# al-mcintyre/mCaller

Measured on AMD Instinct MI355X. Metric: m6A calls/sec (GATC motif, E. coli-like synthetic eventalign), higher is better.
Workload: dtype f64 (K1 window means, everything written); K2 hidden layer f32 + f64 output + f64 re-evaluation near print boundaries (MCALLER_MLP_FP64=1 = f64 throughout: ms_per_step_fp64_mlp); 1 GPU; synthetic 1e+08 eventalign rows per GPU and step, -m GATC, NN classifier (r95 two-base MLP), skip_thresh 0; two resident tables taken in turn, every step a FULL pass (the table declared new: positions + event indices streamed, every row validated); step=full pass, passes_in_flight=4, events_per_gpu=100000000, flush_records_per_gpu=204194, copy_out_bytes_per_pass=8767737

## Files before the change

### include/mcaller_hip.h

```cpp
#ifndef MCALLER_HIP_H
#define MCALLER_HIP_H

#define MC_E_NO_FREE_SLOT (-16)

#include <stdint.h>

#ifdef __cplusplus
extern "C" {
#endif

#define MC_MAX_K 8

#define MC_F_KMER_EQ    0x01
#define MC_F_MODEL_N    0x02
#define MC_F_SEG_START  0x04
#define MC_F_NAME_START 0x08

typedef struct mc_table_view {
    int64_t n_rows;
    const int32_t *pos;
    const int32_t *event_model_e4;
    const int32_t *event_idx;
    const uint8_t *flags;
    int32_t n_seg;
// ... 90 lines not shown
int mc_fastq_read_quality(const char *path, int32_t n_threads, mc_fastq **out);
int64_t mc_fastq_view(const mc_fastq *f, const char **key_pool, const int64_t **key_off, const double **mean);
void mc_fastq_free(mc_fastq *f);

typedef struct mc_ctx mc_ctx;
int mc_ctx_create(int device, mc_ctx **out);
int mc_bind_to_device_numa_node(int device);
void mc_ctx_destroy(mc_ctx *ctx);
int mc_ctx_set_reference(mc_ctx *ctx, const mc_ref_view *host_ref);
int mc_ctx_set_reference_motif(mc_ctx *ctx, const mc_ref_view *host_ref, const char *motif_fwd, const char *repl_fwd, int32_t m_fwd,
                               const char *motif_rev, const char *repl_rev, int32_t m_rev);
int mc_ctx_set_reference_iupac(mc_ctx *ctx, const mc_ref_view *host_ref, const mc_iupac_spec *spec);
int mc_ctx_fetch_reference(mc_ctx *ctx, uint8_t *seq, int64_t n_seq_bytes, uint32_t *mbits_fwd, uint32_t *mbits_rev,
                           int32_t *rank_fwd, int32_t *rank_rev, int64_t n_words, int64_t *site_base, int64_t *n_sites);
int mc_ctx_upload_table(mc_ctx *ctx, const mc_table_view *host_table);
int mc_ctx_set_read_quality(mc_ctx *ctx, const double *qual, int32_t n_reads);

#define MC_TABLE_SLOTS 12
int mc_ctx_reserve_tables(mc_ctx *ctx, int64_t max_rows, int32_t max_segs, int32_t max_reads);
int mc_ctx_upload_table_async(mc_ctx *ctx, const mc_table_view *host_table, const double *read_qual, int32_t *slot);
int mc_ctx_wait_upload(mc_ctx *ctx, int32_t slot);
int mc_ctx_current_slot(mc_ctx *ctx);
int mc_ctx_select_table(mc_ctx *ctx, int32_t slot, int32_t as_new);
int mc_ctx_upload_times_ms(mc_ctx *ctx, int32_t slot, float *h2d_ms, float *validate_ms);
int mc_ctx_parse_times_ms(mc_ctx *ctx, int32_t slot, float *text_h2d_ms, float *parse_ms);
int mc_ctx_set_mlp(mc_ctx *ctx, int32_t n_models, int32_t n_in, int32_t n_hidden,
                   const double *W1, const double *b1, const double *W2, const double *b2,
                   const uint8_t *submodel_of_char);

int mc_ctx_set_forest(mc_ctx *ctx, int32_t n_models, int32_t n_in, const int32_t *model_tree_off,
                      const int32_t *tree_node_off, const int32_t *left, const int32_t *right, const int32_t *feature,
                      const double *threshold, const double *value, const uint8_t *submodel_of_char);

#define MC_CLF_LOGISTIC 1
#define MC_CLF_GNB 2
int mc_ctx_set_simple_classifier(mc_ctx *ctx, int32_t kind, int32_t n_models, int32_t n_in, const double *params, int32_t stride,
                                 const uint8_t *submodel_of_char);

int mc_ctx_set_svm(mc_ctx *ctx, int32_t n_models, int32_t n_in, const int32_t *model_sv_off, const double *sv,
                   const double *dual_coef, const double *params, const uint8_t *submodel_of_char);

typedef struct mc_params {
    int32_t k;
    int32_t skip_thresh;
    double  qual_thresh;
    int32_t tail_contig;
    int32_t score;
    int32_t entry_read;
    int32_t entry_first_idx;
} mc_params;

int mc_last_pass_info(mc_ctx *ctx, int32_t *fused_room, int32_t *rerun);
int mc_ctx_last_scan_mode(mc_ctx *ctx);
int mc_ctx_row_text(mc_ctx *ctx, int32_t on, const char *label_meth, const char *label_unmeth);
int mc_last_row_text(mc_ctx *ctx, const char **text, int64_t *n_bytes, int64_t *n_rows, int32_t *block);
int mc_row_text_release(mc_ctx *ctx, int32_t block);
#define MC_ROWTEXT_PROBE_STRIDE 48
int mc_ctx_rowtext_probe(mc_ctx *ctx, const double *v, int64_t n, const int32_t *fixed, int64_t n_fixed, const double *prob, int64_t n_prob,
                         int32_t shift, char *text, int32_t *len, uint8_t *ok);
int mc_extract_features(mc_ctx *ctx, const mc_params *prm, int64_t *n_records);
int mc_fetch_records(mc_ctx *ctx, const mc_calls_view *host_out);
int mc_fetch_records_view(mc_ctx *ctx, mc_calls_view *out);
int mc_extract_features_async(mc_ctx *ctx, const mc_params *prm);
int mc_wait_records(mc_ctx *ctx, int64_t *n_records, mc_calls_view *out);
int mc_wait_records_begin(mc_ctx *ctx);
int mc_last_times_ms(mc_ctx *ctx, float *out5);
int mc_ctx_set_pass_timing(mc_ctx *ctx, int every_n);
int mc_last_pass_timed(mc_ctx *ctx);
int mc_ctx_sync(mc_ctx *ctx);

int mc_mlp_forward(mc_ctx *ctx, const double *X, const uint8_t *submodel, int64_t n, double *p);
int mc_forest_forward(mc_ctx *ctx, const double *X, const uint8_t *submodel, int64_t n, double *p);
int mc_simple_forward(mc_ctx *ctx, const double *X, const uint8_t *submodel, int64_t n, double *p);
int mc_svm_forward(mc_ctx *ctx, const double *X, const uint8_t *submodel, int64_t n, double *p);

#define MC_UNIQUE_ID_BYTES 128
int64_t mc_site_count(mc_ctx *ctx);
int mc_site_counts(mc_ctx *ctx, int64_t row_offset, int32_t tail_contig, int64_t *n_pending, int64_t *n_cross_contig);
int mc_site_counts_reset(mc_ctx *ctx);
int mc_site_counts_accumulate(mc_ctx *ctx, int64_t row_offset, int32_t tail_contig, int64_t *n_pending, int64_t *n_cross_contig);
int mc_site_counts_add(mc_ctx *ctx, const int64_t *site, const uint8_t *is_meth, const int64_t *first_row, int64_t n);
int mc_comm_available(void);
int mc_comm_unique_id(uint8_t *out128);
int mc_comm_init(mc_ctx *ctx, int32_t world, int32_t rank, const uint8_t *unique_id128);
int mc_comm_destroy(mc_ctx *ctx);
int mc_site_allreduce(mc_ctx *ctx, int32_t *n_meth, int32_t *n_total, int64_t *first_row, float *ms);
int mc_site_counts_fetch(mc_ctx *ctx, int32_t *n_meth, int32_t *n_total, int64_t *first_row);

typedef struct mc_fit_params {
    int32_t n_in, n_hidden;
    int32_t batch_size;
    int32_t max_iter;
    int32_t n_iter_no_change;
    int32_t shuffle;
    double alpha, lr_init, beta1, beta2, epsilon, tol;
    uint64_t seed;
} mc_fit_params;
int mc_mlp_fit(mc_ctx *ctx, const mc_fit_params *prm, const double *X, const uint8_t *y, int64_t n_samples, int32_t n_jobs,
               const int64_t *train_off, const int32_t *train_idx, const int64_t *val_off, const int32_t *val_idx,
               const uint64_t *seeds, const double *init,
               double *W1, double *b1, double *W2, double *b2,
               double *loss_curve , int32_t *n_iter , int64_t *val_correct);

typedef struct mc_forest_params {
    int32_t n_in;
    int32_t n_trees;
// ... 538 lines not shown
```

### mcaller_amd/csrc/mc_dev.h

```cpp
#ifndef MC_DEV_H
#define MC_DEV_H
#include <hip/hip_runtime.h>
#include <hip/hip_ext.h>
#include <sched.h>

#include <algorithm>
#include <cctype>
#include <chrono>
#include <cmath>
#include <cstdio>
#include <cstdlib>
#include <cstring>
#include <type_traits>
#include <vector>

#include "../../include/mcaller_hip.h"

void mc_set_error(const char *fmt, ...);

#define HIP_TRY(expr)                                                                       \
    do {                                                                                    \
        hipError_t _e = (expr);                                                             \
        if (_e != hipSuccess) {                                                             \
            mc_set_error("%s failed: %s (%s:%d)", #expr, hipGetErrorString(_e), __FILE__, __LINE__); \
// ... 289 lines not shown
    const NbDesc *desc;
    Payload *payload;
    long long payload_cap;
    long long *tile_chunk;
    int chunk_shift;
    int shard_shift;
    int shard_mask;
    int32_t *tile_cnt;
    int32_t *tile_half;
    const int32_t *tile_local;
    const int64_t *group_sum;
    int64_t *tile_first;
    DevRecords O;
    Counters *cnt;
    int k, skip_thresh, tail_contig;
    int64_t *rare_list;
    unsigned long long pass_no;
    int32_t *piece_cnt;
    int32_t *piece_kw;
    unsigned long long *chunk_cnt;
};

__device__ __forceinline__ int64_t find_close(const DevTable &T, const NbDesc *__restrict__ desc, int tail_contig,
                                              int nb_abs, int64_t my_end, int64_t r, int &close_pos, bool &close_ns) {
    int64_t rr = r + 1;
    int bb = nb_abs;
    close_ns = false;
    close_pos = 0;
    while (rr < T.n_rows) {
        if (rr < my_end) {
            if (!(T.flags[rr] & MC_F_MODEL_N)) { close_pos = T.pos[rr]; return rr; }
            ++rr;
            continue;
        }
        close_ns = true;
        while (bb + 1 < T.n_nb && T.nb_row_begin[bb + 1] <= rr) ++bb;
        if (desc[bb].filtered) { rr = T.nb_row_begin[bb + 1]; continue; }
        if (!(T.flags[rr] & MC_F_MODEL_N)) { close_pos = T.pos[rr]; return rr; }
        ++rr;
    }
    close_ns = true;
    return tail_contig >= 0 ? T.n_rows : -1;
}

constexpr int PT = 16;
constexpr int NCHUNK = TILE / 64 + 1;
#ifndef MC_CHUNK
#define MC_CHUNK 1024
#endif
constexpr int CHUNK = MC_CHUNK;
constexpr int NCH = TILE / CHUNK;
constexpr int NQ = CHUNK / 512;
static_assert(CHUNK % 512 == 0 && TILE % CHUNK == 0, "whole stripes, whole chunks");

constexpr int GROUP = 1024;

__device__ __forceinline__ int64_t tile_slot(const int32_t *__restrict__ tile_local, const int64_t *__restrict__ group_sum,
                                             int64_t tile, int lane) {
    const int g = (int)(tile / GROUP);
    long long part = 0;
    for (int i = lane; i < g; i += 64) part += group_sum[i];
    for (int o = 32; o > 0; o >>= 1) part += __shfl_xor(part, o);
    return part + tile_local[tile];
}

constexpr int EG = 8;
constexpr int K2_MAXM = 8;

struct PackLayout { size_t pos, seg, info, feats; };
__host__ __device__ inline PackLayout pack_layout(int64_t n, int close32) {
    PackLayout L;
    L.pos = (size_t)n * (close32 ? 4 : 8);
    L.seg = L.pos + (size_t)n * 4;
    L.info = L.seg + (size_t)n * 4;
    L.feats = (L.info + (size_t)n * 4 + 7) & ~(size_t)7;
    return L;
}

struct PackTail { size_t lo32, prob, wmask, hi32, end; };
__host__ __device__ inline PackTail pack_tail(size_t feats_off, size_t m, int k, size_t n_wide) {
    PackTail T;
    T.lo32 = feats_off;
    T.prob = (T.lo32 + m * (size_t)k * 4 + 7) & ~(size_t)7;
    T.wmask = T.prob + m * 8;
    T.hi32 = (T.wmask + m + 3) & ~(size_t)3;
    T.end = T.hi32 + n_wide * 4;
    return T;
}

struct LitArgs {
    DevTable T;
    DevRef R;
    const NbDesc *desc;
    const int64_t *nb_f0;
    const double *qual;
    double qual_thresh;
    int k, skip_thresh, tail_contig, entry_read, entry_first_idx;
    int32_t *run_cnt;
    int32_t *run_rows;
    const int32_t *cnt_local;
    const int64_t *cnt_group;
    const int32_t *rows_local;
    const int64_t *rows_group;
    double *scratch;
    DevRecords L;
    int write;
// ... 90 lines not shown
```

### mcaller_amd/csrc/mc_scan.hip

```cpp
#include "mc_dev.h"

namespace {

__global__ __launch_bounds__(256) void k_unit_columns(DevTable T) {
    const int64_t g4 = blockIdx.x * (int64_t)256 + threadIdx.x;
    const bool have = g4 * 4 < T.n_rows;
    int4 p = make_int4(0, 0, 0, 0);
    if (have) {
        p = *reinterpret_cast<const int4 *>(T.pos + g4 * 4);
        reinterpret_cast<int32_t *>(T.unit_pp)[g4] = (g4 & 1) ? p.w : p.x;
    }
    int before = __shfl_up(p.w, 1);
    if ((threadIdx.x & 63) == 0 && have && g4 > 0) before = T.pos[g4 * 4 - 1];
    const int ps[5] = {before, p.x, p.y, p.z, p.w};
    uint32_t dec = 0, zero = 0;
#pragma unroll
    for (int e = 0; e < 4; ++e) {
        const int64_t r = g4 * 4 + e;
        const bool in = r < T.n_rows;
        dec |= (in && r > 0 && ps[e + 1] < ps[e] ? 1u : 0u) << e;
        zero |= (in && ps[e + 1] == 0 ? 1u : 0u) << e;
    }
    const uint32_t mine = dec | (zero << 8);
    const uint32_t other = __shfl_down(mine, 1);
// ... 207 lines not shown
__device__ __forceinline__ NbDesc desc_uniform(const NbDesc *desc, int b) {
    const NbDesc *p = uniform_ptr(desc) + __builtin_amdgcn_readfirstlane(b);
    union { u32x16 w; NbDesc d; } u;
    asm volatile("s_load_dwordx16 %0, %1, 0x0\n\ts_waitcnt lgkmcnt(0)" : "=s"(u.w) : "s"(p));
    return u.d;
}
__device__ __forceinline__ int64_t desc_row_end_uniform(const NbDesc *desc, int b) {
    const int64_t *p = &(uniform_ptr(desc) + __builtin_amdgcn_readfirstlane(b))->row_end;
    int64_t v;
    asm volatile("s_load_dwordx2 %0, %1, 0x0\n\ts_waitcnt lgkmcnt(0)" : "=s"(v) : "s"(p));
    return v;
}

template <int MODE> constexpr bool summary_cols() { return MODE == SCAN_SUMMARY || MODE == SCAN_VALIDATE_SUMMARY; }
template <int MODE> constexpr bool validating() { return MODE == SCAN_VALIDATE || MODE == SCAN_VALIDATE_SUMMARY; }
template <int MODE> constexpr bool nbits_streamed() { return !summary_cols<MODE>(); }
static_assert(MC_F_MODEL_N == 2, "flag_bytes(): where the bit goes in the flag byte");
__device__ __forceinline__ uint32_t flag_bytes(uint32_t b4) { return (((b4 & 0xFu) * 0x00204081u) & 0x01010101u) << 1; }

template <int MODE>
struct ChunkCols {
    int4 pa[NQ], pb[NQ];
    uint32_t xr[NQ];
    uint32_t pr[NQ];
    uint32_t nb[NQ];
    __device__ __forceinline__ void load(const DevTable &T, int64_t c0, int crows, int lane) {
#pragma unroll
        for (int j = 0; j < NQ; ++j) {
            const int i0 = (j * 64 + lane) * 8;
            pa[j] = pb[j] = make_int4(0, 0, 0, 0);
            xr[j] = pr[j] = 0u;
            nb[j] = 0xFFu;
            if (i0 < crows) {
                if (summary_cols<MODE>()) {
                    const int2 pp = T.unit_pp[(c0 + i0) >> 3];
                    pa[j].x = pp.x;
                    pb[j].w = pp.y;
                    if (MODE == SCAN_VALIDATE_SUMMARY) {
                        xr[j] = T.xrel[(c0 + i0) >> 3];
                        pr[j] = T.prel[(c0 + i0) >> 3];
                    }
                } else {
                    pa[j] = *reinterpret_cast<const int4 *>(T.pos + c0 + i0);
                    pb[j] = *reinterpret_cast<const int4 *>(T.pos + c0 + i0 + 4);
                    nb[j] = T.nbits[(c0 + i0) >> 3];
                    if (MODE == SCAN_VALIDATE) {
                        xr[j] = T.xrel[(c0 + i0) >> 3];
                    }
                }
            }
        }
    }
};

struct DenseStash { const int4 *pa, *pb, *fw; const int *dec; };
__device__ __forceinline__ void dense_block_rows(const K1Args &A, TileSlots &S, long long &ahead, DenseStash L, int nb_abs, int64_t c0,
                                                 int64_t c1, int2 tail_p, uint32_t tail_f) {
    const DevTable &T = A.T;
    const int lane = threadIdx.x, k = A.k;
    const unsigned long long below = (1ull << lane) - 1ull;
    const uint32_t kmask = (1u << k) - 1u;
    ScanGlobals G;
    G.pos = T.pos; G.flags = T.flags; G.nb_row_begin = T.nb_row_begin; G.desc = A.desc; G.n_rows = T.n_rows;
    G.n_nb = T.n_nb; G.tail_contig = A.tail_contig; G.k = k; G.skip_thresh = A.skip_thresh;
    const NbDesc d = desc_uniform(A.desc, nb_abs);
    if (d.mode != MODE_REGULAR) return;
    const uint32_t *gbits = (d.rev ? A.R.mr : A.R.mf) + d.mask_off;
    if (d.extra_row() >= c0 && d.extra_row() < c1) {
        const CloseRes xc = far_close_body(G, nb_abs, d.row_end, d.extra_row());
        Payload P;
        P.r = d.extra_row(); P.close_row = xc.row; P.m = d.extra_mpos; P.close_pos = xc.pos;
        P.flags = PF_EXTRA | (xc.ns ? PF_CLOSE_NS : 0u);
        P.nb = nb_abs;
        S.put(lane == 0 && xc.row >= 0, P, &ahead);
    }
    const int64_t lb_abs = max(d.row_begin, d.first());
    const int lo = (int)(max(lb_abs, c0) - c0), hi = (int)(min(d.row_end, c1) - c0);
    const int hi_close = (int)(min(d.row_end, c1 + 2) - c0);
    const uint32_t base_flags = (d.stray_q != NO_STRAY ? PF_STRAY : 0u) | (d.rev ? PF_REV : 0u);
#pragma unroll 1
    for (int j = 0; j < NQ; ++j) {
        if (j * 512 + 512 <= lo || j * 512 >= hi) continue;
        const int i0 = (j * 64 + lane) * 8;
        const int4 qa = L.pa[j * 64 + lane], qb = L.pb[j * 64 + lane], qw = L.fw[j * 64 + lane];
        const int un = j * 64 + lane + 1;
        const bool last = un >= NQ * 64;
        const int4 na = L.pa[last ? 0 : un], nw = L.fw[last ? 0 : un];
        const int nx = last ? tail_p.x : na.x, ny = last ? tail_p.y : na.y;
        const uint32_t nf = last ? tail_f : (uint32_t)nw.x;
        const int ps[10] = {qa.x, qa.y, qa.z, qa.w, qb.x, qb.y, qb.z, qb.w, nx, ny};
        const uint32_t nbits = ((uint32_t)qw.x & 0xFFu) | ((nf & 3u) << 8);
        const uint32_t below_hi = (1u << min(max(hi - i0, 0), 10)) - 1u, from_lo = ~((1u << min(max(lo - i0, 0), 10)) - 1u);
        const uint32_t act = below_hi & from_lo & ~nbits & 0xFFu;
        const uint32_t free_rows = ((1u << min(max(hi_close - i0, 0), 10)) - 1u) & ~nbits;
        const uint32_t dc1 = free_rows >> 1, dc2 = ~dc1 & (nbits >> 1) & (free_rows >> 2);
        const bool w_any = L.dec[j * 64 + lane] != 0;
        const int w_base = ps[0] & ~31;
        const uint64_t W = ((uint64_t)(uint32_t)qw.w << 32) | (uint32_t)qw.z;
        auto site_off = [&](int p, bool &ok) -> int {
            const uint32_t q = (uint32_t)(p - w_base);
            const bool beyond = p >= d.contig_len;
            ok = beyond | (w_any & (q <= (uint32_t)(64 - k)));
            const uint32_t bits = beyond ? 0u : (uint32_t)(W >> (q & 63u)) & kmask;
            return __ffs(bits) - 1;
        };
        uint32_t cbits = 0, farbits = 0, multibits = 0, how = 0;
// ... 39 lines not shown
        const int rank0 = S.total + before;
        const int cs = A.chunk_shift;
        const long long slot0 = S.slot_of(rank0);
        const int room = rank0 < PT ? PT - rank0 : (1 << cs) - ((rank0 - PT) & ((1 << cs) - 1));
#pragma unroll
        for (int e = 0; e < 8; ++e) {
            if (!((cbits >> e) & 1u) || ((farbits >> e) & 1u)) continue;
            const uint32_t h = (how >> (4 * e)) & 15u;
            const int dc = 1 + (int)(h >> 3);
            Payload P;
            P.r = c0 + i0 + e; P.close_row = c0 + i0 + e + dc; P.m = ps[e] + (int)(h & 7u);
            P.close_pos = dc == 1 ? ps[e + 1] : ps[e + 2];
            P.flags = base_flags | (((multibits >> e) & 1u) ? PF_MULTI : 0u);
            P.nb = nb_abs;
            const int t = __popc(cbits & ((1u << e) - 1u));
            const long long slot = t < room ? (slot0 < 0 ? -1 : slot0 + t) : S.slot_of(rank0 + t);
            if (slot >= 0) A.payload[slot] = P;
            __builtin_amdgcn_sched_barrier(0);
        }
        if (__ballot((cbits & farbits) != 0u)) {
            for (uint32_t fb = cbits & farbits; fb; fb &= fb - 1u) {
                const int e = __ffs(fb) - 1;
                const RowRes fr = far_row_body(G, gbits, d.contig_len, nb_abs, d.row_end, c0 + i0 + e);
                Payload P;
                P.r = c0 + i0 + e; P.close_row = fr.cr; P.m = fr.m; P.close_pos = fr.cp;
                P.flags = fr.pf | base_flags;
                P.nb = nb_abs;
                const long long slot = S.slot_of(rank0 + __popc(cbits & ((1u << e) - 1u)));
                if (slot >= 0) A.payload[slot] = P;
            }
        }
        S.total += n_new;
    }
}

#ifdef MC_SCAN_WPE
#define MC_SCAN_ATTR __attribute__((amdgpu_waves_per_eu(MC_SCAN_WPE, MC_SCAN_WPE)))
#else
#define MC_SCAN_ATTR __attribute__((amdgpu_waves_per_eu(MODE == SCAN_SUMMARY ? 6 : 1)))
#endif
template <int CG, int MODE>
__global__ __launch_bounds__(64) MC_SCAN_ATTR void k1_scan(K1Args A) {
    __shared__ __attribute__((aligned(16))) CandUnit s_cand[CG];
    __shared__ long long s_chunk[NCHUNK];
    const DevTable &T = A.T;
    const int lane = threadIdx.x;
    const int64_t tile = blockIdx.x;
    const int k = A.k;
    const int64_t t0 = tile * TILE;
    const int nrows = (int)(min(t0 + (int64_t)TILE, T.n_rows) - t0);
    const unsigned long long below = (1ull << lane) - 1ull;
    const uint32_t kmask = (1u << k) - 1u;

    ChunkCols<MODE> C;
    C.load(T, t0, min(nrows, CHUNK), lane);
    int2 tail_p = make_int2(0, 0);
    uint32_t tail_f = 0;
    auto load_tail = [&](int64_t c1) {
        tail_p = make_int2(T.pos[c1], T.pos[c1 + 1]);
        tail_f = ((((uint32_t)T.nbits[(c1 >> 3) + 1] << 8) | (uint32_t)T.nbits[c1 >> 3]) >> (int)(c1 & 7)) & 3u;
    };
    if constexpr (CG > 64) load_tail(t0 + min(nrows, CHUNK));
    int before_p = 0;
    if (MODE == SCAN_VALIDATE && t0 > 0) before_p = T.pos[t0 - 1];
    int nb0 = __builtin_amdgcn_readfirstlane(T.tile_nb[tile]);
    ScanGlobals G;
    G.pos = T.pos; G.flags = T.flags; G.nb_row_begin = T.nb_row_begin; G.desc = A.desc; G.n_rows = T.n_rows;
    G.n_nb = T.n_nb; G.tail_contig = A.tail_contig; G.k = k; G.skip_thresh = A.skip_thresh;
    TileSlots S{A, tile, s_chunk, 0, lane};
    long long ahead = -1;
    if constexpr (CG > 64) ahead = S.take_ahead();
    int half = 0;
    static_assert(CG <= 64 || NCH == 2, "tile_half: two chunks per tile");

#pragma unroll 1
    for (int ch = 0; ch < NCH; ++ch) {
        const int crows = min(nrows - ch * CHUNK, CHUNK);
        if (crows <= 0) break;
        const int64_t c0 = t0 + (int64_t)ch * CHUNK, c1 = c0 + crows;
        const bool more = ch + 1 < NCH && nrows > (ch + 1) * CHUNK;
        while (nb0 + 1 < T.n_nb && desc_row_end_uniform(A.desc, nb0) <= c0) ++nb0;
        const NbDesc da = desc_uniform(A.desc, nb0);
        const bool has_b = nb0 + 1 < T.n_nb && da.row_end < c1;
        const NbDesc db = desc_uniform(A.desc, nb0 + (has_b ? 1 : 0));
        const bool has_c = has_b && nb0 + 2 < T.n_nb && db.row_end < c1;
        const int nfast = has_b ? 2 : 1;

        uint32_t mlo[NQ], mhi[NQ];
        bool decidable[NQ];
        auto fetch_mask_words = [&]() {
            const bool rega = da.mode == MODE_REGULAR, regb = has_b && db.mode == MODE_REGULAR;
            const int loa = (int)(max(max(da.row_begin, da.first()), c0) - c0), hia = (int)(min(da.row_end, c1) - c0);
            const int lob = (int)(max(max(db.row_begin, db.first()), c0) - c0), hib = (int)(min(db.row_end, c1) - c0);
            const uint32_t *ga = (da.rev ? A.R.mr : A.R.mf) + da.mask_off, *gb = (db.rev ? A.R.mr : A.R.mf) + db.mask_off;
            const int nwa = ((da.contig_len + 31) >> 5) + 2, nwb = ((db.contig_len + 31) >> 5) + 2;
#pragma unroll
            for (int j = 0; j < NQ; ++j) {
                const int i0 = (j * 64 + lane) * 8;
                const int p0 = C.pa[j].x, p7 = C.pb[j].w;
                const bool ina = rega && i0 >= loa && i0 + 8 <= hia, inb = regb && i0 >= lob && i0 + 8 <= hib;
                const uint32_t span = (uint32_t)p7 - (uint32_t)p0 + (uint32_t)k;
                const int w = p0 >> 5;
                decidable[j] = (ina || inb) && span - 1u < 32u && p0 >= 0 && w + 1 < (ina ? nwa : nwb);
                const uint32_t *g = (inb ? gb : ga) + (decidable[j] ? w : 0);
                mlo[j] = g[0];
                mhi[j] = g[1];
            }
        };
        if (CG <= 64 || MODE != SCAN_VALIDATE) fetch_mask_words();

        if (validating<MODE>()) {
            for (int bi = 0; bi < nfast; ++bi) {
                const int64_t rb = bi ? db.row_begin : da.row_begin, re = bi ? db.row_end : da.row_end;
                const uint32_t vf_known = bi ? db.vf : da.vf;
                const int vlo = (int)(max(rb, c0) - c0), vhi = (int)(min(re, c1) - c0);
                const int pred_from = rb < c0 ? 0 : vlo + 1;
                int n_pdec = 0, n_inc = 0, n_dec = 0, n_pairs = 0, n_pos0 = 0;
                uint32_t f_cut = 0;
#pragma unroll
                for (int j = 0; j < NQ; ++j) {
                    if (j * 512 + 512 <= vlo || j * 512 >= vhi) continue;
                    const int i0 = (j * 64 + lane) * 8;
                    const bool whole = i0 >= pred_from && i0 + 8 <= vhi;
                    const bool cut = !whole && i0 + 8 > vlo && i0 < vhi;
                    if (MODE == SCAN_VALIDATE_SUMMARY) {
                        if (whole) {
// ... 66 lines not shown
#if !defined(MC_DENSE_PREFETCH) || !MC_DENSE_PREFETCH
            if (more) {
                C.load(T, c0 + CHUNK, min(nrows - (ch + 1) * CHUNK, CHUNK), lane);
                load_tail(c0 + CHUNK + min(nrows - (ch + 1) * CHUNK, CHUNK));
            }
#endif
        } else {
        int ncand = 0, seg_end_a = 0;
        bool overflow = false;
        for (int bi = 0; bi < nfast; ++bi) {
            const bool reg = (bi ? db.mode : da.mode) == MODE_REGULAR;
            if (reg) {
                const int64_t lb_abs = bi ? max(db.row_begin, db.first()) : max(da.row_begin, da.first());
                const int lo = (int)(max(lb_abs, c0) - c0), hi = (int)(min(bi ? db.row_end : da.row_end, c1) - c0);
#pragma unroll
                for (int j = 0; j < NQ; ++j) {
                    if (j * 512 + 512 <= lo || j * 512 >= hi) continue;
                    const int i0 = (j * 64 + lane) * 8;
                    const int p0 = C.pa[j].x, p7 = C.pb[j].w;
                    const bool touches = i0 + 8 > lo && i0 < hi;
                    const int span = p7 - p0 + k;
                    const uint32_t bits = bits_from(mlo[j], mhi[j], p0 & 31) & (0xFFFFFFFFu >> ((32 - span) & 31));
                    const bool cand = touches && (!decidable[j] || bits != 0u);
                    const unsigned long long bal = __ballot(cand);
                    if (!bal) continue;
                    if (ncand + __popcll(bal) > CG) { overflow = true; continue; }
                    int nx = 0, ny = 0;
                    uint32_t nf = 0x3u;
                    if (!summary_cols<MODE>()) {
                        nx = __shfl_down(C.pa[j].x, 1);
                        ny = __shfl_down(C.pa[j].y, 1);
                        nf = __shfl_down(C.nb[j], 1);
                        if (j + 1 < NQ) {
                            const int sx = __shfl(C.pa[(j + 1) % NQ].x, 0), sy = __shfl(C.pa[(j + 1) % NQ].y, 0);
                            const uint32_t sf = __shfl(C.nb[(j + 1) % NQ], 0);
                            if (lane == 63) { nx = sx; ny = sy; nf = sf; }
                        }
                    }
                    if (cand) {
                        CandUnit *g = s_cand + (ncand + __popcll(bal & below));
                        int4 *gp = reinterpret_cast<int4 *>(g);
                        if (!summary_cols<MODE>()) {
                            gp[0] = C.pa[j];
                            gp[1] = C.pb[j];
                            gp[2] = make_int4(nx, ny, (int)flag_bytes(C.nb[j]), (int)flag_bytes(C.nb[j] >> 4));
                        }
                        gp[3] = make_int4((int)((flag_bytes(nf) & 0xFFFFu) | ((uint32_t)i0 << 16)), (int)mlo[j], (int)mhi[j], decidable[j] ? (p0 >> 5) : -1);
                    }
                    ncand += __popcll(bal);
                }
            }
            if (bi == 0) seg_end_a = ncand;
        }
        if (more) C.load(T, c0 + CHUNK, min(nrows - (ch + 1) * CHUNK, CHUNK), lane);
        if (overflow) {
            scan_blocks_slowly(A, nb0, nfast, c0, c1, S, lane);
        } else {
            __syncthreads();
            if (!nbits_streamed<MODE>()) {
                for (int base = 0; base < ncand; base += 64) {
                    const int gi = base + lane;
                    if (gi < ncand) {
                        CandUnit *g = s_cand + gi;
                        const int i0 = (int)(reinterpret_cast<const uint32_t *>(g)[12] >> 16);
                        const uint8_t *fr = T.flags + c0 + i0;
                        const uint2 f8 = *reinterpret_cast<const uint2 *>(fr);
                        const uint32_t nf = *reinterpret_cast<const uint16_t *>(fr + 8);
                        if (summary_cols<MODE>()) {
                            const int32_t *pr = T.pos + c0 + i0;
                            const int4 a = *reinterpret_cast<const int4 *>(pr), b4 = *reinterpret_cast<const int4 *>(pr + 4);
                            const int2 nx = *reinterpret_cast<const int2 *>(pr + 8);
                            int4 *gp = reinterpret_cast<int4 *>(g);
                            gp[0] = a;
                            gp[1] = b4;
                            reinterpret_cast<int2 *>(g)[4] = nx;
                        }
                        reinterpret_cast<uint2 *>(g)[5] = f8;
                        reinterpret_cast<uint32_t *>(g)[12] = nf | ((uint32_t)i0 << 16);
                    }
                }
                __syncthreads();
            }

            for (int bi = 0; bi < nfast; ++bi) {
                const int nb_abs = nb0 + bi;
                const int first_g = bi ? seg_end_a : 0, seg_end = bi ? ncand : seg_end_a;
                const NbDesc d = desc_uniform(A.desc, nb_abs);
                if (d.mode != MODE_REGULAR) continue;
                const uint32_t *gbits = (d.rev ? A.R.mr : A.R.mf) + d.mask_off;
                auto site_off = [&](const CandUnit *g, int p, bool &ok) -> int {
                    const int wb = (int)g->mw[2], wi = (p >> 5) - wb, sh = p & 31;
                    const uint32_t two = bits_from(g->mw[0], g->mw[1], sh), one = g->mw[1] >> sh;
                    ok = wb >= 0 && (wi == 0 || (wi == 1 && sh + k <= 32));
                    const uint32_t bits = (wi == 0 ? two : one) & kmask;
                    int o = bits ? (int)__builtin_ctz(bits) : -1;
                    if (p >= d.contig_len) { o = -1; ok = true; }
                    return o;
                };
                if (d.extra_row() >= c0 && d.extra_row() < c1) {
                    const CloseRes xc = far_close(G, nb_abs, d.row_end, d.extra_row());
                    Payload P;
                    P.r = d.extra_row(); P.close_row = xc.row; P.m = d.extra_mpos; P.close_pos = xc.pos;
                    P.flags = PF_EXTRA | (xc.ns ? PF_CLOSE_NS : 0u);
                    P.nb = nb_abs;
                    S.put(lane == 0 && xc.row >= 0, P);
                }
                const int64_t lb_abs = max(d.row_begin, d.first());
// ... 153 lines not shown
```

### mcaller_amd/csrc/mc_stream.hip

```cpp
#include "mc_ctx.h"

static int ensure_pinned(mc_ctx *c, int64_t n, int k) {
    if (c->H.capacity >= n && c->h_k == k) return 0;
    c->H = DevRecords();
    const int64_t cap = std::max<int64_t>(n + n / 4, 1 << 16);
    const size_t bytes[6] = {(size_t)cap * k * 8, (size_t)cap * 4, (size_t)cap * 4, (size_t)cap * 8, (size_t)cap * 4, (size_t)cap * 8};
    for (int i = 0; i < 6; ++i)
        if (int rc = c->H_pin[i].alloc(bytes[i])) return rc;
    c->H.feats = c->H_pin[0].get<double>(); c->H.site_pos = c->H_pin[1].get<int32_t>(); c->H.site_seg = c->H_pin[2].get<int32_t>();
    c->H.close_row = c->H_pin[3].get<int64_t>(); c->H.info = c->H_pin[4].get<uint32_t>(); c->H.prob = c->H_pin[5].get<double>();
    c->H.capacity = cap;
    c->h_k = k;
    return 0;
}

static int copy_out_features(mc_ctx *c, int64_t n, int k, hipStream_t st) {
    HIP_TRY(hipMemcpyAsync(c->H.feats, c->O.feats, (size_t)n * k * 8, hipMemcpyDeviceToHost, st));
    HIP_TRY(hipMemcpyAsync(c->H.site_pos, c->O.site_pos, (size_t)n * 4, hipMemcpyDeviceToHost, st));
    HIP_TRY(hipMemcpyAsync(c->H.site_seg, c->O.site_seg, (size_t)n * 4, hipMemcpyDeviceToHost, st));
    HIP_TRY(hipMemcpyAsync(c->H.close_row, c->O.close_row, (size_t)n * 8, hipMemcpyDeviceToHost, st));
    HIP_TRY(hipMemcpyAsync(c->H.info, c->O.info, (size_t)n * 4, hipMemcpyDeviceToHost, st));
    return 0;
}

// ... 598 lines not shown
        c->in_rerun = true;
        const int rc = mc_extract_features(c, &b.prm, &n);
        c->in_rerun = false;
        c->T = T_now; c->qual = const_cast<double *>(q_now); c->n_qual = nq_now; c->cur = cur_now;
        if (rc) return rc;
        c->last_timed = 1;
        *n_records = n;
        return mc_fetch_records_view(c, out);
    }
    const int64_t n = (int64_t)st.n_records;
    c->last_timed = (b.used && b.timed) ? 1 : 0;
    if (b.used && b.timed) {
        float t_k0 = 0, t_scan = 0, t_emit = 0, t_k2 = 0;
        HIP_TRY(hipEventElapsedTime(&t_k0, b.ev[EV_K0_START], b.ev[EV_SCAN_START]));
        if (b.emit_aside && MC_EVENTS_ON_KERNELS) {
            HIP_TRY(hipEventElapsedTime(&t_scan, b.ev[EV_SCAN_START], b.ev[EV_LIST_END]));
            HIP_TRY(hipEventElapsedTime(&t_emit, b.ev[EV_EMIT_START], b.ev[EV_EMIT_END]));
        } else {
            HIP_TRY(hipEventElapsedTime(&t_scan, b.ev[EV_SCAN_START], b.ev[EV_EMIT_END]));
            t_emit = 0.0f;
        }
        HIP_TRY(hipEventElapsedTime(&t_k2, b.ev[EV_K2_START], b.one_kernel ? b.ev[EV_DONE] : b.ev[EV_K2_END]));
        c->times[0] = t_k0; c->times[1] = t_scan; c->times[2] = t_emit; c->times[3] = t_k2;
        c->times[4] = t_k0 + t_scan + t_emit + t_k2;
    }
    c->O = b.B.O;
    c->last_n = n;
    c->last_slots = b.fused_room > 0 ? std::min<int64_t>(b.slots, b.cap) : n;
    c->last_k = b.k ? b.k : c->last_k;
    *n_records = n;
    out->capacity = n;
    out->feats = b.H.feats; out->site_pos = b.H.site_pos; out->site_seg = b.H.site_seg;
    out->close_row = b.H.close_row; out->info = b.H.info; out->prob = b.H.prob;
    out->close_row32 = b.h_close32;
    out->call_row = nullptr;
    out->compacted = 1;
    const bool packed = n > 0 && b.used;
    out->feats_lo32 = packed ? b.h_lo32 : nullptr;
    out->feats_hi32 = packed ? b.h_hi32 : nullptr;
    out->feats_wide = packed ? b.h_wmask : nullptr;
    out->n_wide = packed ? b.h_n_wide : 0;
    out->n_call_rows = n > 0 && b.used ? b.h_n_calls : 0;
    return 0;
}

extern "C" int mc_last_pass_info(mc_ctx *c, int32_t *fused_room, int32_t *rerun) {
    if (fused_room) *fused_room = c->last_fused_room;
    if (rerun) *rerun = c->last_rerun;
    return 0;
}

extern "C" int mc_ctx_last_scan_mode(mc_ctx *c) { return c->last_scan_mode; }

extern "C" int mc_ctx_set_pass_timing(mc_ctx *c, int every_n) {
    if (every_n < 0) { mc_set_error("mc_ctx_set_pass_timing: every_n < 0"); return -12; }
    c->timing_every = every_n;
    return 0;
}

extern "C" int mc_last_pass_timed(mc_ctx *c) { return c->last_timed; }

extern "C" int mc_last_times_ms(mc_ctx *c, float *out5) {
    for (int i = 0; i < 5; ++i) out5[i] = c->times[i];
    return 0;
}

static int classifier_forward(mc_ctx *c, int which, const double *X, const uint8_t *submodel, int64_t n, double *p) {
    HIP_TRY(hipSetDevice(c->device));
    if (which != c->clf.kind) {
        mc_set_error("classifier forward: no %s set", which == 1 ? "forest" : (which == 2 ? "logistic / naive Bayes model" : (which == 3 ? "SVM" : "MLP")));
        return -12;
    }
    if (n <= 0) return 0;
    double *dX = nullptr, *dp = nullptr;
    uint8_t *ds = nullptr;
    const int ni = c->clf.n_in;
    Pool pool("classifier forward");
    if (pool.get(&dX, (size_t)n * ni) || pool.get(&dp, (size_t)n) || pool.get(&ds, (size_t)n)) return -10;
    HIP_TRY(hipMemcpyAsync(dX, X, (size_t)n * ni * 8, hipMemcpyHostToDevice, c->stream));
    HIP_TRY(hipMemcpyAsync(ds, submodel, (size_t)n, hipMemcpyHostToDevice, c->stream));
    HIP_TRY(hipMemsetAsync(dp, 0xFF, (size_t)n * 8, c->stream));
    launch_classifier(c, c->stream, dX, ni - 1, (const int32_t *)nullptr, (const int32_t *)nullptr, (const double *)nullptr,
                      (const uint32_t *)nullptr, ds, n, dp, (const unsigned long long *)nullptr, (const unsigned int *)nullptr);
    HIP_TRY(hipMemcpyAsync(p, dp, (size_t)n * 8, hipMemcpyDeviceToHost, c->stream));
    HIP_TRY(hipStreamSynchronize(c->stream));
    HIP_TRY(hipGetLastError());
    return 0;
}

extern "C" int mc_mlp_forward(mc_ctx *c, const double *X, const uint8_t *submodel, int64_t n, double *p) {
    return classifier_forward(c, 0, X, submodel, n, p);
}

extern "C" int mc_forest_forward(mc_ctx *c, const double *X, const uint8_t *submodel, int64_t n, double *p) {
    return classifier_forward(c, 1, X, submodel, n, p);
}

extern "C" int mc_simple_forward(mc_ctx *c, const double *X, const uint8_t *submodel, int64_t n, double *p) {
    return classifier_forward(c, 2, X, submodel, n, p);
}

extern "C" int mc_svm_forward(mc_ctx *c, const double *X, const uint8_t *submodel, int64_t n, double *p) {
    return classifier_forward(c, 3, X, submodel, n, p);
}

namespace {
// ... 158 lines not shown
```

### mcaller_amd/device.py

```python
import ctypes as C
import os

import numpy as np

from . import _lib
from ._lib import Params, Records, check, last_error, lib, make_ref_view, _ptr


def default_device_index():
    for var in ('MCALLER_DEVICE', 'LOCAL_RANK'):
        if os.environ.get(var, '') != '':
            return int(os.environ[var])
    return 0


def _serialized(fn):
    import functools

    @functools.wraps(fn)
    def call(self, *a, **kw):
        with self._lock:
            return fn(self, *a, **kw)
    return call

# ... 321 lines not shown
    ROWTEXT_PROBE_FILL = 0xA5

    @_serialized
    def rowtext_probe(self, values=(), fixed=(), prob=(), shift=0):
        v = np.ascontiguousarray(values, dtype=np.float64)
        f = np.ascontiguousarray(fixed, dtype=np.int32)
        p = np.ascontiguousarray(prob, dtype=np.float64)
        n_all = len(v) + len(f) + len(p)
        text = np.empty((n_all, self.ROWTEXT_PROBE_STRIDE), dtype=np.uint8)
        length = np.empty(n_all, dtype=np.int32)
        ok = np.empty(n_all, dtype=np.uint8)
        check(lib().mc_ctx_rowtext_probe(self._ctx, _ptr(v), len(v), _ptr(f), len(f), _ptr(p), len(p), int(shift), _ptr(text), _ptr(length),
                                         _ptr(ok)))
        return text, length, ok.astype(bool)

    @_serialized
    def fetch(self, copy=True):
        n, k = self._last
        if not copy:
            v = _lib.CallsView()
            check(lib().mc_fetch_records_view(self._ctx, C.byref(v)))
            return Records.from_view(v, n, k, self)
        rec = Records(n, k)
        v = rec.view()
        check(lib().mc_fetch_records(self._ctx, C.byref(v)))
        rec.n = n
        return rec

    def extract(self, k, skip_thresh, qual_thresh, **kw):
        self.run(k, skip_thresh, qual_thresh, **kw)
        return self.fetch()

    @_serialized
    def sync(self):
        check(lib().mc_ctx_sync(self._ctx))

    @_serialized
    def set_pass_timing(self, every_n):
        check(lib().mc_ctx_set_pass_timing(self._ctx, int(every_n)))

    @_serialized
    def last_pass_timed(self):
        return bool(lib().mc_last_pass_timed(self._ctx))

    @_serialized
    def last_pass_info(self):
        a, b = C.c_int32(0), C.c_int32(0)
        check(lib().mc_last_pass_info(self._ctx, C.byref(a), C.byref(b)))
        return a.value, bool(b.value)

    @_serialized
    def last_scan_mode(self):
        return int(lib().mc_ctx_last_scan_mode(self._ctx))

    @_serialized
    def times_ms(self):
        t = np.zeros(5, dtype=np.float32)
        check(lib().mc_last_times_ms(self._ctx, _ptr(t)))
        return dict(strand_resolve=float(t[0]), window_scan=float(t[1]), emit=float(t[2]), classifier=float(t[3]),
                    total=float(t[4]))

    @staticmethod
    def comm_unique_id():
        buf = np.zeros(128, dtype=np.uint8)
        check(lib().mc_comm_unique_id(_ptr(buf)))
        return buf.tobytes()

    @staticmethod
    def comm_probe():
        check(lib().mc_comm_available())

    @_serialized
    def site_counts_fetch(self):
        n = lib().mc_site_count(self._ctx)
        n_meth, n_total = np.zeros(n, dtype=np.int32), np.zeros(n, dtype=np.int32)
        first = np.full(n, np.iinfo(np.int64).max, dtype=np.int64)
        check(lib().mc_site_counts_fetch(self._ctx, _ptr(n_meth), _ptr(n_total), _ptr(first)))
        return n_meth, n_total, first

    @_serialized
    def comm_init(self, world, rank, unique_id):
        uid = np.frombuffer(unique_id, dtype=np.uint8).copy()
        assert len(uid) == 128
        check(lib().mc_comm_init(self._ctx, int(world), int(rank), _ptr(uid)))

    @_serialized
    def comm_destroy(self):
        lib().mc_comm_destroy(self._ctx)

    @_serialized
    def site_counts(self, row_offset=0, tail_contig=-1):
        pending, cross = C.c_int64(0), C.c_int64(0)
        check(lib().mc_site_counts(self._ctx, int(row_offset), int(tail_contig), C.byref(pending), C.byref(cross)))
        self.n_cross_contig = cross.value
        return pending.value

    @_serialized
    def site_counts_reset(self):
        check(lib().mc_site_counts_reset(self._ctx))

    @_serialized
    def site_counts_accumulate(self, row_offset=0, tail_contig=-1):
        pending, cross = C.c_int64(0), C.c_int64(0)
        check(lib().mc_site_counts_accumulate(self._ctx, int(row_offset), int(tail_contig), C.byref(pending), C.byref(cross)))
        self.n_cross_contig = cross.value
        return pending.value
# ... 617 lines not shown
```

Measured before the change: 800.4 million calls/s.

## Add whole-tile fast scan path when a tile lies inside one regular block

```diff
diff --git a/include/mcaller_hip.h b/include/mcaller_hip.h
--- a/include/mcaller_hip.h
+++ b/include/mcaller_hip.h
@@ -166,6 +166,7 @@
 
 int mc_last_pass_info(mc_ctx *ctx, int32_t *fused_room, int32_t *rerun);
 int mc_ctx_last_scan_mode(mc_ctx *ctx);
+int64_t mc_ctx_whole_tiles(mc_ctx *ctx, uint8_t *per_tile);
 int mc_ctx_row_text(mc_ctx *ctx, int32_t on, const char *label_meth, const char *label_unmeth);
 int mc_last_row_text(mc_ctx *ctx, const char **text, int64_t *n_bytes, int64_t *n_rows, int32_t *block);
 int mc_row_text_release(mc_ctx *ctx, int32_t block);
diff --git a/mcaller_amd/csrc/mc_dev.h b/mcaller_amd/csrc/mc_dev.h
--- a/mcaller_amd/csrc/mc_dev.h
+++ b/mcaller_amd/csrc/mc_dev.h
@@ -365,6 +365,13 @@
 constexpr int NCH = TILE / CHUNK;
 constexpr int NQ = CHUNK / 512;
 static_assert(CHUNK % 512 == 0 && TILE % CHUNK == 0, "whole stripes, whole chunks");
+
+constexpr int NQT = TILE / 512;
+
+__host__ __device__ inline bool scan_tile_is_whole(const NbDesc &d, int64_t t0, int nrows) {
+    if (nrows != TILE || d.row_begin >= t0 || d.row_end < t0 + TILE) return false;
+    return d.mode != MODE_REGULAR || (d.first() >= 0 && d.first() <= t0);
+}
 
 constexpr int GROUP = 1024;
 
diff --git a/mcaller_amd/csrc/mc_scan.hip b/mcaller_amd/csrc/mc_scan.hip
--- a/mcaller_amd/csrc/mc_scan.hip
+++ b/mcaller_amd/csrc/mc_scan.hip
@@ -283,6 +283,176 @@
         }
     }
 };
+
+__device__ __forceinline__ int32_t i32_uniform(const int32_t *p) {
+    int32_t v;
+    asm volatile("s_load_dword %0, %1, 0x0\n\ts_waitcnt lgkmcnt(0)" : "=s"(v) : "s"(uniform_ptr(p)));
+    return v;
+}
+
+template <int MODE>
+struct TileCols {
+    int2 pp[NQT];
+    uint32_t xr[NQT], pr[NQT];
+    __device__ __forceinline__ void load(const DevTable &T, int64_t t0, int nrows, int lane) {
+#pragma unroll
+        for (int j = 0; j < NQT; ++j) {
+            const int i0 = (j * 64 + lane) * 8;
+            pp[j] = make_int2(0, 0);
+            xr[j] = pr[j] = 0u;
+            if (i0 < nrows) {
+                pp[j] = T.unit_pp[(t0 + i0) >> 3];
+                if (MODE == SCAN_VALIDATE_SUMMARY) {
+                    xr[j] = T.xrel[(t0 + i0) >> 3];
+                    pr[j] = T.prel[(t0 + i0) >> 3];
+                }
+            }
+        }
+    }
+};
+template <int MODE>
+__device__ __forceinline__ void take_chunk(ChunkCols<MODE> &C, const TileCols<MODE> &W, int ch) {
+#pragma unroll
+    for (int j = 0; j < NQ; ++j) {
+        C.pa[j] = C.pb[j] = make_int4(0, 0, 0, 0);
+        C.pa[j].x = W.pp[ch * NQ + j].x;
+        C.pb[j].w = W.pp[ch * NQ + j].y;
+        C.xr[j] = W.xr[ch * NQ + j];
+        C.pr[j] = W.pr[ch * NQ + j];
+        C.nb[j] = 0xFFu;
+    }
+}
+
+template <int CG, int MODE>
+__device__ __forceinline__ bool scan_whole_tile(const K1Args &A, const ScanGlobals &G, TileSlots &S, CandUnit *s_cand, const TileCols<MODE> &W,
+                                                const NbDesc &d, int nb_abs, int64_t t0, int lane) {
+    static_assert(TILE <= 65536 && NQT * 64 * 8 == TILE, "CandUnit::i0 holds a tile-relative row");
+    const DevTable &T = A.T;
+    const int k = A.k;
+    const unsigned long long below = (1ull << lane) - 1ull;
+    const uint32_t kmask = (1u << k) - 1u;
+    const bool reg = d.mode == MODE_REGULAR;
+    const uint32_t *gbits = (d.rev ? A.R.mr : A.R.mf) + d.mask_off;
+    const int nw = ((d.contig_len + 31) >> 5) + 2;
+    uint32_t mlo[NQT], mhi[NQT];
+    bool decidable[NQT];
+#pragma unroll
+    for (int j = 0; j < NQT; ++j) {
+        const int p0 = W.pp[j].x, p7 = W.pp[j].y;
+        const uint32_t span = (uint32_t)p7 - (uint32_t)p0 + (uint32_t)k;
+        const int w = p0 >> 5;
+        decidable[j] = reg && span - 1u < 32u && p0 >= 0 && w + 1 < nw;
+        const uint32_t *g = gbits + (decidable[j] ? w : 0);
+        mlo[j] = g[0];
+        mhi[j] = g[1];
+    }
+    if (MODE == SCAN_VALIDATE_SUMMARY) {
+        uint32_t any_p = 0u, any_x = 0u, all_x = 0xFFu;
+#pragma unroll
+        for (int j = 0; j < NQT; ++j) {
+            any_p |= W.pr[j];
+            any_x |= W.xr[j];
+            all_x &= W.xr[j] | (W.xr[j] >> 8);
+        }
+        const uint32_t seen = (__ballot((any_p & 0xFFu) != 0u) ? V_POS_DEC : 0u) | (__ballot((any_x & 0xFFu) != 0u) ? V_IDX_INC : 0u) |
+                              (__ballot((any_x >> 8) != 0u) ? V_IDX_DEC : 0u) | (__ballot((all_x & 0xFFu) != 0xFFu) ? V_IDX_EQ : 0u) |
+                              (__ballot((any_p >> 8) != 0u) ? V_POS0 : 0u);
+        if ((seen & ~d.vf) && lane == 0) note_validation(A, nb_abs, seen);
+    }
+    if (!reg) return true;
+    int ncand = 0;
+#pragma unroll
+    for (int j = 0; j < NQT; ++j) {
+        const int i0 = (j * 64 + lane) * 8;
+        const int p0 = W.pp[j].x, p7 = W.pp[j].y;
+        const int span = p7 - p0 + k;
+        const uint32_t bits = bits_from(mlo[j], mhi[j], p0 & 31) & (0xFFFFFFFFu >> ((32 - span) & 31));
+        const bool cand = !decidable[j] || bits != 0u;
+        const unsigned long long bal = __ballot(cand);
+        if (ncand + __popcll(bal) > CG) return false;
+        if (cand) {
+            int4 *gp = reinterpret_cast<int4 *>(s_cand + (ncand + __popcll(bal & below)));
+            gp[3] = make_int4((int)((uint32_t)i0 << 16), (int)mlo[j], (int)mhi[j], decidable[j] ? (p0 >> 5) : -1);
+        }
+        ncand += __popcll(bal);
+    }
+    if (ncand == 0) return true;
+    __builtin_amdgcn_fence(__ATOMIC_ACQ_REL, "wavefront");
+    static_assert(CG <= 64, "one lane per listed unit");
+    if (lane < ncand) {
+        CandUnit *g = s_cand + lane;
+        const int i0 = (int)(reinterpret_cast<const uint32_t *>(g)[12] >> 16);
+        const uint8_t *fr = T.flags + t0 + i0;
+        const int32_t *pr = T.pos + t0 + i0;
+        const uint2 f8 = *reinterpret_cast<const uint2 *>(fr);
+        const uint32_t nf = *reinterpret_cast<const uint16_t *>(fr + 8);
+        const int4 a = *reinterpret_cast<const int4 *>(pr), b4 = *reinterpret_cast<const int4 *>(pr + 4);
+        const int2 nx = *reinterpret_cast<const int2 *>(pr + 8);
+        int4 *gp = reinterpret_cast<int4 *>(g);
+        gp[0] = a;
+        gp[1] = b4;
+        reinterpret_cast<int2 *>(g)[4] = nx;
+        reinterpret_cast<uint2 *>(g)[5] = f8;
+        reinterpret_cast<uint32_t *>(g)[12] = nf | ((uint32_t)i0 << 16);
+    }
+    __builtin_amdgcn_fence(__ATOMIC_ACQ_REL, "wavefront");
+    auto site_off = [&](const CandUnit *g, int p, bool &ok) -> int {
+        const int wb = (int)g->mw[2], wi = (p >> 5) - wb, sh = p & 31;
+        const uint32_t two = bits_from(g->mw[0], g->mw[1], sh), one = g->mw[1] >> sh;
+        ok = wb >= 0 && (wi == 0 || (wi == 1 && sh + k <= 32));
+        const uint32_t bits = (wi == 0 ? two : one) & kmask;
+        int o = bits ? (int)__builtin_ctz(bits) : -1;
+        if (p >= d.contig_len) { o = -1; ok = true; }
+        return o;
+    };
+    const uint32_t base_flags = (d.stray_q != NO_STRAY ? PF_STRAY : 0u) | (d.rev ? PF_REV : 0u);
+    for (int base = 0; base < ncand * 8; base += 64) {
+        const int idx = base + lane;
+        const bool have = idx < ncand * 8;
+        const CandUnit *g = s_cand + (have ? idx >> 3 : 0);
+        const int e = idx & 7;
+        const int p = g->pos[e], p1 = g->pos[e + 1], p2 = g->pos[e + 2];
+        const uint32_t f = g->fl[e], f1 = g->fl[e + 1], f2 = g->fl[e + 2];
+        const int i = (int)g->i0 + e;
+        bool closed = false, far = false;
+        int m = 0, cp = 0;
+        int64_t cr = 0;
+        uint32_t pf = 0;
+        if (have && !(f & MC_F_MODEL_N)) {
+            bool ok;
+            const int o = site_off(g, p, ok);
+            if (!ok) far = true;
+            else if (o >= 0) {
+                m = p + o;
+                int c = -1;
+                if (i + 1 < TILE && !(f1 & MC_F_MODEL_N)) { c = i + 1; cp = p1; }
+                else if (i + 2 < TILE && (f1 & MC_F_MODEL_N) && !(f2 & MC_F_MODEL_N)) { c = i + 2; cp = p2; }
+                if (c >= 0) {
+                    cr = t0 + c;
+                    closed = cp > m;
+                    if (closed && cp <= m + A.skip_thresh + 1) {
+                        bool ok2;
+                        const int o2 = site_off(g, cp, ok2);
+                        if (!ok2) far = true;
+                        else if (o2 > 0) pf |= PF_MULTI;
+                    }
+                } else far = true;
+            }
+        }
+        if (__ballot(far)) {
+            if (far) {
+                const RowRes fr = far_row(G, gbits, d.contig_len, nb_abs, d.row_end, t0 + i);
+                closed = fr.closed; m = fr.m; cp = fr.cp; cr = fr.cr; pf = fr.pf;
+            }
+        }
+        Payload P;
+        P.r = t0 + i; P.close_row = cr; P.m = m; P.close_pos = cp;
+        P.flags = pf | base_flags;
+        P.nb = nb_abs;
+        S.put(closed, P);
+    }
+    return true;
+}
 
 struct DenseStash { const int4 *pa, *pb, *fw; const int *dec; };
 __device__ __forceinline__ void dense_block_rows(const K1Args &A, TileSlots &S, long long &ahead, DenseStash L, int nb_abs, int64_t c0,
@@ -428,8 +598,14 @@
     const unsigned long long below = (1ull << lane) - 1ull;
     const uint32_t kmask = (1u << k) - 1u;
 
+    constexpr bool WHOLE = CG <= 64 && summary_cols<MODE>();
+    static_assert(!WHOLE || NCH == 2, "take_chunk(C, W, 1): two chunks per tile");
+    TileCols<MODE> W;
     ChunkCols<MODE> C;
-    C.load(T, t0, min(nrows, CHUNK), lane);
+    if constexpr (WHOLE) {
+        W.load(T, t0, nrows, lane);
+        take_chunk(C, W, 0);
+    } else C.load(T, t0, min(nrows, CHUNK), lane);
     int2 tail_p = make_int2(0, 0);
     uint32_t tail_f = 0;
     auto load_tail = [&](int64_t c1) {
@@ -439,7 +615,9 @@
     if constexpr (CG > 64) load_tail(t0 + min(nrows, CHUNK));
     int before_p = 0;
     if (MODE == SCAN_VALIDATE && t0 > 0) before_p = T.pos[t0 - 1];
-    int nb0 = __builtin_amdgcn_readfirstlane(T.tile_nb[tile]);
+    int nb0;
+    if constexpr (WHOLE) nb0 = i32_uniform(T.tile_nb + tile);
+    else nb0 = __builtin_amdgcn_readfirstlane(T.tile_nb[tile]);
     ScanGlobals G;
     G.pos = T.pos; G.flags = T.flags; G.nb_row_begin = T.nb_row_begin; G.desc = A.desc; G.n_rows = T.n_rows;
     G.n_nb = T.n_nb; G.tail_contig = A.tail_contig; G.k = k; G.skip_thresh = A.skip_thresh;
@@ -448,6 +626,15 @@
     if constexpr (CG > 64) ahead = S.take_ahead();
     int half = 0;
     static_assert(CG <= 64 || NCH == 2, "tile_half: two chunks per tile");
+
+    if constexpr (WHOLE) {
+        NbDesc d0 = desc_uniform(A.desc, nb0);
+        while (nb0 + 1 < T.n_nb && d0.row_end <= t0) d0 = desc_uniform(A.desc, ++nb0);
+        if (scan_tile_is_whole(d0, t0, nrows) && scan_whole_tile<CG, MODE>(A, G, S, s_cand, W, d0, nb0, t0, lane)) {
+            if (lane == 0) A.tile_cnt[tile] = S.total;
+            return;
+        }
+    }
 
 #pragma unroll 1
     for (int ch = 0; ch < NCH; ++ch) {
@@ -620,7 +807,10 @@
             }
             if (bi == 0) seg_end_a = ncand;
         }
-        if (more) C.load(T, c0 + CHUNK, min(nrows - (ch + 1) * CHUNK, CHUNK), lane);
+        if (more) {
+            if constexpr (WHOLE) take_chunk(C, W, 1);
+            else C.load(T, c0 + CHUNK, min(nrows - (ch + 1) * CHUNK, CHUNK), lane);
+        }
         if (overflow) {
             scan_blocks_slowly(A, nb0, nfast, c0, c1, S, lane);
         } else {
diff --git a/mcaller_amd/csrc/mc_stream.hip b/mcaller_amd/csrc/mc_stream.hip
--- a/mcaller_amd/csrc/mc_stream.hip
+++ b/mcaller_amd/csrc/mc_stream.hip
@@ -674,6 +674,31 @@
 
 extern "C" int mc_ctx_last_scan_mode(mc_ctx *c) { return c->last_scan_mode; }
 
+extern "C" int64_t mc_ctx_whole_tiles(mc_ctx *c, uint8_t *per_tile) {
+    HIP_TRY(hipSetDevice(c->device));
+    const DevTable &T = c->T;
+    if (c->cur < 0 || !c->sync.K.desc || T.n_nb <= 0 || T.n_nb > c->scratch_nb || T.n_tiles <= 0) {
+        mc_set_error("mc_ctx_whole_tiles: no table, or no synchronous pass over it yet");
+        return -12;
+    }
+    HIP_TRY(hipStreamSynchronize(c->stream));
+    std::vector<NbDesc> desc((size_t)T.n_nb);
+    std::vector<int32_t> tile_nb((size_t)T.n_tiles);
+    HIP_TRY(hipMemcpy(desc.data(), c->sync.K.desc, desc.size() * sizeof(NbDesc), hipMemcpyDeviceToHost));
+    HIP_TRY(hipMemcpy(tile_nb.data(), T.tile_nb, tile_nb.size() * sizeof(int32_t), hipMemcpyDeviceToHost));
+    int64_t n = 0;
+    for (int64_t tile = 0; tile < T.n_tiles; ++tile) {
+        const int64_t t0 = tile * TILE;
+        int nb = tile_nb[(size_t)tile];
+        if (nb < 0 || nb >= T.n_nb) { mc_set_error("mc_ctx_whole_tiles: tile %lld begins in block %d", (long long)tile, nb); return -12; }
+        while (nb + 1 < T.n_nb && desc[(size_t)nb].row_end <= t0) ++nb;
+        const bool whole = scan_tile_is_whole(desc[(size_t)nb], t0, (int)(std::min<int64_t>(t0 + TILE, T.n_rows) - t0));
+        if (per_tile) per_tile[tile] = whole ? 1 : 0;
+        n += whole;
+    }
+    return n;
+}
+
 extern "C" int mc_ctx_set_pass_timing(mc_ctx *c, int every_n) {
     if (every_n < 0) { mc_set_error("mc_ctx_set_pass_timing: every_n < 0"); return -12; }
     c->timing_every = every_n;
diff --git a/mcaller_amd/device.py b/mcaller_amd/device.py
--- a/mcaller_amd/device.py
+++ b/mcaller_amd/device.py
@@ -397,6 +397,14 @@
     @_serialized
     def last_scan_mode(self):
         return int(lib().mc_ctx_last_scan_mode(self._ctx))
+
+    @_serialized
+    def whole_tiles(self, n_rows):
+        out = np.zeros((n_rows + 2047) // 2048, dtype=np.uint8)
+        n = int(lib().mc_ctx_whole_tiles(self._ctx, _ptr(out)))
+        check(min(n, 0))
+        assert n == int(out.sum())
+        return out.astype(bool)
 
     @_serialized
     def times_ms(self):
```

Result: faster. 856.8 million calls/s (median of 6 runs) (+7.0%).
